# leggedrobotics/wild_visual_navigation

Hardware: AMD Instinct MI355X
Metric: frames/sec (448x448 DINO-ViT-S/8 + seg + MLP train-step) (higher is better)
Workload: dtype fp16 + e5m2-MX-correction linears (a w = a_h w_h + 2^-12 (a_h8 w_l8 + a_l8 w_h8); ~16 significand bits per product) + f16 attention products (two-plane q in the first six blocks), fp32 accumulate / residual (<= 1e-3 parity mode)

## Files before the change

### include/wvn_hip.h

```cpp
#ifndef WVN_HIP_H
#define WVN_HIP_H
#include <stddef.h>
#ifdef __cplusplus
extern "C" {
#endif

#define WVN_MAX_DEPTH 32
#define WVN_PREC_F32 0
#define WVN_PREC_BF16 1
#define WVN_PREC_X3 2
#define WVN_PREC_FP8 3
#define WVN_PREC_F16 4

#define WVN_PREC_MIX 5

int wvn_version(void);

#define WVN_VIT_MLP_FUSED 1
#define WVN_VIT_QKV_FUSED 2
#define WVN_VIT_FUSE_ANY_SIZE 4
#define WVN_VIT_NO_PROJ_IN_MLP 8
#define WVN_VIT_NO_LN_HANDOVER 16
#define WVN_VIT_NO_A384_X3 32
#define WVN_VIT_X3_NO_A384 64
// ... 251 lines not shown
int wvn_pixel_mlp_pack(const wvn_mlp_desc* d, const float* params, void* packed, void* stream);
int wvn_pixel_mlp_infer(const wvn_mlp_desc* d, const void* packed, void* zx, int ldzx, int batch, int grid, int out_h,
                        int out_w, float mean, float std, float std_factor, const float* conf_state, float* trav,
                        float* conf, float* loss_reco, void* stream);

size_t wvn_pixel_mlp_exact_pack_bytes(const wvn_mlp_desc* d);
size_t wvn_pixel_mlp_exact_workspace_bytes(const wvn_mlp_desc* d, int batch, int grid);
int wvn_pixel_mlp_exact_pack(const wvn_mlp_desc* d, const float* params, void* packed, void* stream);
int wvn_pixel_mlp_infer_exact(const wvn_mlp_desc* d, const float* params, const void* packed, const float* tokens,
                              int ld_tokens, int batch, int grid, int out_h, int out_w, float mean, float std,
                              float std_factor, const float* conf_state, float* trav, float* conf, float* loss_reco,
                              void* workspace, size_t workspace_bytes, void* stream);

size_t wvn_segment_predict_workspace_bytes(const wvn_mlp_desc* d, int B, int S);
int wvn_segment_predict(const wvn_mlp_desc* d, const float* params, const float* feat, int ld_row, long long ld_frame,
                        int B, int S, const void* seg, int seg_bytes, int H, int W, float mean, float std, float std_factor,
                        const float* conf_state, float* trav, float* conf, float* loss_reco, void* workspace,
                        size_t workspace_bytes, void* stream);

size_t wvn_wire_bytes(int H, int W, int S, int D);
int wvn_wire_pack(const void* seg, int seg_is_i64, const float* feat, int ldf, void* out, int H, int W, int S, int D, void* stream);
int wvn_wire_unpack(const void* in, long long* seg_i64, int* seg_i32, float* feat, int H, int W, int S, int D, void* stream);

int wvn_debug_gemm_bf16_timed(const void* A, int lda, const void* W, int ldw, const float* bias, void* C, int ldc, int M,
                              int N, int K, int epi, long long* dbg, void* stream);
int wvn_debug_gemm_a384_x3(const void* A, const void* A_lo, int lda, const void* W, const void* W_lo, const float* bias, void* C,
                           void* C_lo, int ldc, int M, int N, int epi, long long* dbg, void* stream);
int wvn_debug_gemm_n384_x3(const void* A, const void* A_lo, int lda, const void* W, const void* W_lo, const float* bias, const float* ls,
                           float* C, int ldc, int M, int K, long long* dbg, void* stream);
int wvn_debug_mlp_x3_frag(const void* xn, const void* xn_lo, const void* W1, const void* W1_lo, const float* b1, void* hid, void* hid_lo,
                          const void* W2p, const float* b2, float* x, int M, int F, long long* dbg1, long long* dbg2, void* stream);
int wvn_debug_gemm_n384_mx(const void* A_h, const void* A_l8, const void* A_h8, const void* Wp, const float* bias, const float* ls, float* C,
                           int ldc, int M, int K, long long* dbg, void* stream);
int wvn_debug_mlp_mx(const float* x, int ldx, const float* ln_stats, const float* ln_g, const float* ln_b, const void* W1p, const float* b1,
                     void* hid_h, void* hid_l8, void* hid_h8, const void* W2p, const float* b2, float* xout, int M, int F, long long* dbg1,
                     long long* dbg2, void* stream);
int wvn_debug_qkv_mx(const float* x, int ldx, const float* ln_stats, const float* ln_g, const float* ln_b, const void* Wp, const float* bias, void* q,
                     void* q_lo, void* k, void* vt, int heads, int npad, int ntok_s, float q_scale, int M, long long* dbg, void* stream);
int wvn_debug_f16_saturate(const float* in, void* out_f16, int n, void* stream);
int wvn_debug_attention_timing(long long* dbg);
int wvn_debug_attention_variant(int variant);
int wvn_debug_attention_planes(const void* q, const void* q_lo, const void* k, const void* vt, void* out, void* out_lo, int B, int heads,
                               int ntok, int ntok_s, int npad, int out_frag, int qsplit_form, void* stream);
int wvn_debug_n384_pair(int on);
int wvn_debug_kmeans_assign_form(int form);
int wvn_debug_kmeans_linear_rows(int rows);

int wvn_debug_kmeans_screen_stats(unsigned long long* out, int reset);
int wvn_debug_qkv_fused_timing(long long* dbg);
int wvn_debug_mlp_fused_timing(long long* dbg);
int wvn_debug_gemm_n384(const void* A, int lda, const void* W, int ldw, const float* bias, float* C, int ldc, int M, int K,
                        void* stream);


size_t wvn_dense_crf_workspace_bytes(int B, int H, int W, int K);
int wvn_dense_crf(const float* logits1, int K1, long long s1b, long long s1c, long long s1p, const float* logits2, int K2, long long s2b,
                  long long s2c, long long s2p, const unsigned char* image, int B, int H, int W, int iterations, float pos_w, float pos_xy_std,
                  float bi_w, float bi_xy_std, float bi_rgb_std, int* labels, int* nseg_last, float* probs, float* debug, void* workspace,
                  size_t workspace_bytes, void* stream);
int wvn_crf_image(const void* frame, int frame_u8, int B, int src_h, int src_w, const int* rows, const int* cols, int out_h, int out_w,
                  unsigned char* out, void* stream);

size_t wvn_dense_crf_permutohedral_workspace_bytes(int B, int H, int W, int K);
int wvn_dense_crf_permutohedral(const float* logits1, int K1, long long s1b, long long s1c, long long s1p, const float* logits2, int K2,
                                long long s2b, long long s2c, long long s2p, const unsigned char* image, int B, int H, int W, int iterations,
                                float pos_w, float pos_xy_std, float bi_w, float bi_xy_std, float bi_rgb_std, int* labels, int* nseg_last,
// ... 12 lines not shown
```

### wild_visual_navigation_amd/_lib.py

```python
import ctypes as C
import os
import threading

import torch

_HERE = os.path.dirname(os.path.abspath(__file__))
LIB_PATH = os.environ.get("WVN_LIB_PATH") or os.path.join(_HERE, "lib", "libwvn_hip.so")
if os.environ.get("WVN_LIB_PATH"):
    import sys as _sys

    print(f"[wild_visual_navigation_amd] WVN_LIB_PATH is set: loading {LIB_PATH} instead of the in-tree build", file=_sys.stderr)

WVN_MAX_DEPTH = 32
PREC_F32, PREC_BF16, PREC_X3, PREC_FP8, PREC_F16, PREC_MIX = 0, 1, 2, 3, 4, 5
VIT_MLP_FUSED = 1
VIT_QKV_FUSED = 2
VIT_FUSE_ANY_SIZE = 4
VIT_NO_PROJ_IN_MLP = 8
VIT_NO_LN_HANDOVER = 16
VIT_NO_A384_X3 = 32
VIT_NO_MX = 1024


def vit_qsplit_blocks(n: int) -> int:
# ... 33 lines not shown
        ("mlp_dim", C.c_int), ("precision", C.c_int), ("flags", C.c_int),
        ("patch_w", C.c_void_p), ("patch_b", C.c_void_p), ("cls_pos", C.c_void_p), ("pos", C.c_void_p),
        ("norm_g", C.c_void_p), ("norm_b", C.c_void_p),
        ("layers", VitLayer * WVN_MAX_DEPTH),
    ]


class MlpDesc(C.Structure):
    _fields_ = [("D", C.c_int), ("H1", C.c_int), ("H2", C.c_int), ("reserved", C.c_int)]


_lib = None
_lock = threading.Lock()

_i, _f, _p, _ll, _sz = C.c_int, C.c_float, C.c_void_p, C.c_longlong, C.c_size_t
_SIGNATURES = {
    "wvn_version": ([], _i),
    "wvn_vit_workspace_bytes": ([_p, _i], _sz),
    "wvn_vit_forward": ([_p, _p, _i, _p, _p, _i, _p, _sz, _p], _i),
    "wvn_vit_forward_u8": ([_p, _p, _i, _p, _p, _i, _p, _sz, _p], _i),
    "wvn_vit_forward_frames": ([_p, _p, _i, _i, _i, _p, _p, _i, _p, _p, _i, _p, _sz, _p], _i),
    "wvn_vit_forward_frames_pair": ([_p, _p, _i, _i, _i, _p, _p, _p, _i, _p, _p, _i, _p, _sz, _p], _i),
    "wvn_resize_nearest_crop": ([_p, _p, _ll, _i, _i, _p, _p, _i, _i, _i, _p], _i),
    "wvn_prof_enable": ([_i], _i),
    "wvn_prof_collect": ([_p, _p], _i),
    "wvn_gemm_bf16": ([_p, _i, _p, _i, _p, _p, _i, _i, _i, _i, _i, _p], _i),
    "wvn_debug_attention_variant": ([_i], _i),
    "wvn_debug_attention_planes": ([_p, _p, _p, _p, _p, _p, _i, _i, _i, _i, _i, _i, _i, _p], _i),
    "wvn_debug_kmeans_assign_form": ([_i], _i),
    "wvn_debug_kmeans_screen_stats": ([_p, _i], _i),
    "wvn_debug_mlp_x3_frag": ([_p, _p, _p, _p, _p, _p, _p, _p, _p, _p, _i, _i, _p, _p, _p], _i),
    "wvn_debug_gemm_n384_x3": ([_p, _p, _i, _p, _p, _p, _p, _p, _i, _i, _i, _p, _p], _i),
    "wvn_debug_gemm_n384_mx": ([_p, _p, _p, _p, _p, _p, _p, _i, _i, _i, _p, _p], _i),
    "wvn_debug_mlp_mx": ([_p, _i, _p, _p, _p, _p, _p, _p, _p, _p, _p, _p, _p, _i, _i, _p, _p, _p], _i),
    "wvn_debug_qkv_mx": ([_p, _i, _p, _p, _p, _p, _p, _p, _p, _p, _p, _i, _i, _i, _f, _i, _p, _p], _i),
    "wvn_debug_gemm_a384_x3": ([_p, _p, _i, _p, _p, _p, _p, _p, _i, _i, _i, _i, _p, _p], _i),
    "wvn_stream_create_cu_mask": ([_p, _p, _i], _i),
    "wvn_stream_destroy": ([_p], _i),
    "wvn_debug_qkv_fused_timing": ([_p], _i),
    "wvn_debug_mlp_fused_timing": ([_p], _i),
    "wvn_qkv_fused": ([_p, _i, _p, _p, _f, _p, _p, _p, _p, _p, _i, _i, _i, _f, _i, _p], _i),
    "wvn_proj_mlp_fused": ([_p, _i, _p, _p, _p, _p, _p, _f, _p, _p, _p, _p, _p, _p, _i, _i, _i, _p], _i),
    "wvn_mlp_fused": ([_p, _i, _p, _p, _f, _p, _p, _p, _p, _p, _p, _i, _i, _i, _p], _i),
    "wvn_gemm_f16": ([_p, _i, _p, _i, _p, _p, _i, _i, _i, _i, _i, _p], _i),
    "wvn_qkv_fused_f16": ([_p, _i, _p, _p, _f, _p, _p, _p, _p, _p, _i, _i, _i, _f, _i, _p], _i),
    "wvn_proj_mlp_resident": ([_p, _i, _p, _p, _p, _p, _f, _p, _p, _p, _p, _p, _i, _i, _i, _p, _p, _f, _p, _p], _i),
    "wvn_proj_mlp_resident_f16": ([_p, _i, _p, _p, _p, _p, _f, _p, _p, _p, _p, _p, _i, _i, _i, _p, _p, _f, _p, _p], _i),
    "wvn_qkv_prenorm": ([_p, _p, _p, _p, _p, _p, _i, _i, _i, _f, _i, _p], _i),
    "wvn_qkv_prenorm_f16": ([_p, _p, _p, _p, _p, _p, _i, _i, _i, _f, _i, _p], _i),
    "wvn_proj_mlp_fused_f16": ([_p, _i, _p, _p, _p, _p, _p, _f, _p, _p, _p, _p, _p, _p, _i, _i, _i, _p], _i),
    "wvn_mlp_fused_f16": ([_p, _i, _p, _p, _f, _p, _p, _p, _p, _p, _p, _i, _i, _i, _p], _i),
    "wvn_attention_f16": ([_p, _p, _p, _p, _i, _i, _i, _i, _f, _p], _i),
    "wvn_gemm_x3": ([_p, _p, _i, _p, _p, _i, _p, _p, _p, _i, _i, _i, _i, _i, _p], _i),
    "wvn_quantize_rows_fp8": ([_p, _i, _i, _p, _i, _p, _i, _i, _p], _i),
    "wvn_layernorm_fp8": ([_p, _p, _p, _p, _i, _p, _i, _i, _f, _p], _i),
    "wvn_gemm_fp8": ([_p, _i, _p, _i, _p, _p, _p, _p, _i, _i, _i, _i, _i, _p], _i),
    "wvn_gemm_a768_fp8": ([_p, _i, _p, _p, _p, _p, _p, _p, _i, _i, _i, _i, _p, _p, _p, _i, _i, _i, _f, _p], _i),
    "wvn_gemm_fp8_mx": ([_p, _i, _p, _p, _i, _p, _p, _p, _p, _i, _i, _i, _i, _i, _p], _i),
    "wvn_split_planes": ([_p, _i, _p, _p, _i, _i, _i, _p], _i),
    "wvn_attention_x3": ([_p, _p, _p, _p, _p, _p, _p, _p, _i, _i, _i, _i, _f, _p], _i),
    "wvn_gemm_f32": ([_p, _i, _i, _p, _i, _i, _p, _p, _i, _i, _i, _i, _i, _p, _i, _p], _i),
    "wvn_layernorm": ([_p, _p, _p, _p, _i, _i, _i, _f, _p], _i),
    "wvn_attention_bf16": ([_p, _p, _p, _p, _i, _i, _i, _i, _f, _p], _i),
    "wvn_attention_f32": ([_p, _p, _p, _p, _i, _i, _i, _i, _f, _p], _i),
    "wvn_patchify": ([_p, _p, _i, _i, _i, _i, _p], _i),
    "wvn_patchify_u8": ([_p, _p, _i, _i, _i, _p], _i),
# ... 109 lines not shown
```

### wild_visual_navigation_amd/csrc/api.hip

```cpp
#include <math.h>
#include <string.h>

#include "../../include/wvn_hip.h"

#include "common.h"
#include "wvn_internal.h"

#define RET_IF(x)            \
  do {                       \
    int rc__ = (x);          \
    if (rc__ != WVN_OK) return rc__; \
  } while (0)

extern "C" {

int wvn_version(void) { return 100; }

size_t wvn_vit_workspace_bytes(const wvn_vit_model* m, int batch) {
  if (!m || batch <= 0) return 0;
  return wvn_vit_workspace_bytes_impl(m, batch);
}

int wvn_vit_forward(const wvn_vit_model* m, const float* img, int batch, float* tokens_f32, void* tokens_lowp,
                    int ld_lowp, void* workspace, size_t workspace_bytes, void* stream) {
// ... 175 lines not shown
int wvn_debug_qkv_fused_timing(long long* dbg) { g_qkv_fused_dbg = dbg; return WVN_OK; }
int wvn_stream_create_cu_mask(void** stream, const unsigned int* mask, int words) {
  if (!stream || !mask || words <= 0) return WVN_ERR_ARG;
  hipStream_t st = nullptr;
  const hipError_t e = hipExtStreamCreateWithCUMask(&st, (uint32_t)words, mask);
  if (e != hipSuccess) return (int)e;
  *stream = (void*)st;
  return WVN_OK;
}
int wvn_stream_destroy(void* stream) {
  if (!stream) return WVN_ERR_ARG;
  const hipError_t e = hipStreamDestroy((hipStream_t)stream);
  return e == hipSuccess ? WVN_OK : (int)e;
}

int wvn_debug_gemm_a384_x3(const void* A, const void* A_lo, int lda, const void* W, const void* W_lo, const float* bias, void* C,
                           void* C_lo, int ldc, int M, int N, int epi, long long* dbg, void* stream) {
  if (epi != EPI_GELU_BF16 && epi != EPI_RESID_F32) return WVN_ERR_ARG;
  return wvn_gemm_a384_x3_launch(wvn_desc_a384(A, A_lo, lda, W, W_lo, bias, C, C_lo, ldc, M, N, dbg), epi, (hipStream_t)stream);
}
int wvn_debug_gemm_n384_x3(const void* A, const void* A_lo, int lda, const void* W, const void* W_lo, const float* bias, const float* ls,
                           float* C, int ldc, int M, int K, long long* dbg, void* stream) {
  return wvn_gemm_n384_x3_launch(wvn_desc_n384(A, A_lo, lda, W, W_lo, bias, ls, C, ldc, M, K, nullptr, dbg), EPI_RESID_F32, (hipStream_t)stream);
}
int wvn_debug_mlp_x3_frag(const void* xn, const void* xn_lo, const void* W1, const void* W1_lo, const float* b1, void* hid, void* hid_lo,
                          const void* W2p, const float* b2, float* x, int M, int F, long long* dbg1, long long* dbg2, void* stream) {
  RET_IF(wvn_gemm_a384_x3_launch(wvn_desc_a384(xn, xn_lo, 384, W1, W1_lo, b1, hid, hid_lo, F, M, F, dbg1), EPI_GELU_FRAG, (hipStream_t)stream));
  return wvn_gemm_n384_x3_frag_launch(wvn_desc_n384(hid, hid_lo, F, W2p, nullptr, b2, nullptr, x, 384, M, F, nullptr, dbg2), EPI_RESID_F32, (hipStream_t)stream);
}
int wvn_debug_gemm_n384_mx(const void* A_h, const void* A_l8, const void* A_h8, const void* Wp, const float* bias, const float* ls, float* C,
                           int ldc, int M, int K, long long* dbg, void* stream) {
  return wvn_gemm_n384_mx_launch(wvn_desc_n384(A_h, A_l8, K, Wp, nullptr, bias, ls, C, ldc, M, K, nullptr, dbg, A_h8), EPI_RESID_F32, (hipStream_t)stream);
}
int wvn_debug_mlp_mx(const float* x, int ldx, const float* ln_stats, const float* ln_g, const float* ln_b, const void* W1p, const float* b1,
                     void* hid_h, void* hid_l8, void* hid_h8, const void* W2p, const float* b2, float* xout, int M, int F, long long* dbg1,
                     long long* dbg2, void* stream) {
  GemmBf16Params p1 = wvn_desc_a384(nullptr, nullptr, 0, W1p, nullptr, b1, hid_h, hid_l8, F, M, F, dbg1, hid_h8);
  wvn_desc_ln_on_load(p1, x, ldx, ln_stats, ln_g, ln_b);
  RET_IF(wvn_gemm_a384_mx_launch(p1, EPI_GELU_FRAG, (hipStream_t)stream));
  if (!W2p) return WVN_OK;
  return wvn_gemm_n384_mx_launch(wvn_desc_n384(hid_h, hid_l8, F, W2p, nullptr, b2, nullptr, xout, 384, M, F, nullptr, dbg2, hid_h8), EPI_RESID_F32, (hipStream_t)stream);
}
int wvn_debug_qkv_mx(const float* x, int ldx, const float* ln_stats, const float* ln_g, const float* ln_b, const void* Wp, const float* bias, void* q,
                     void* q_lo, void* k, void* vt, int heads, int npad, int ntok_s, float q_scale, int M, long long* dbg, void* stream) {
  GemmBf16Params p = wvn_desc_a384(nullptr, nullptr, 0, Wp, nullptr, bias, nullptr, nullptr, 0, M, 3 * heads * 64, dbg);
  wvn_desc_ln_on_load(p, x, ldx, ln_stats, ln_g, ln_b);
  wvn_desc_qkv_epilogue(p, q, k, vt, heads, npad, 0, ntok_s, q_scale, 1, q_lo);
  return wvn_gemm_a384_mx_launch(p, EPI_QKV, (hipStream_t)stream);
}
int wvn_debug_n384_pair(int on) {
  if (on >= 32) { wvn_gemm_a384_mx_set_form(on - 32); return WVN_OK; }
  wvn_gemm_n384_x3_set_pair(on);
  return WVN_OK;
}
int wvn_debug_kmeans_screen_stats(unsigned long long* out, int reset) { return out ? wvn_kmeans_pixels_screen_stats(out, reset) : WVN_ERR_ARG; }
int wvn_debug_kmeans_assign_form(int form) { wvn_kmeans_pixels_set_assign_form(form); return WVN_OK; }
int wvn_debug_attention_variant(int v) { wvn_attention_bf16_set_variant(v); wvn_attention_bf16_set_variant_f16(v); return WVN_OK; }
int wvn_debug_attention_planes(const void* q, const void* q_lo, const void* k, const void* vt, void* out, void* out_lo, int B, int heads, int ntok,
                               int ntok_s, int npad, int out_frag, int qsplit_form, void* stream) {
  if (!q || !k || !vt || !out || B < 1 || heads < 1 || ntok < 1 || ntok_s < ntok || ntok_s > npad) return WVN_ERR_ARG;
  if (qsplit_form < 0 || qsplit_form > 2 || (qsplit_form == 0) != (q_lo == nullptr)) return WVN_ERR_ARG;
  if (out_frag < 0 || out_frag > 2 || (out_frag != 0 && (!out_lo || heads != 6))) return WVN_ERR_ARG;
  return wvn_attention_bf16_launch_f16((const bf16_t*)q, (const bf16_t*)k, (const bf16_t*)vt, (bf16_t*)out, B, heads, ntok, ntok_s, npad, 0.f,
                                       (hipStream_t)stream, (bf16_t*)out_lo, (const bf16_t*)q_lo, out_frag, qsplit_form);
}

int wvn_debug_gemm_bf16_timed(const void* A, int lda, const void* W, int ldw, const float* bias, void* C, int ldc, int M,
                              int N, int K, int epi, long long* dbg, void* stream) {
  if (epi < 0 || epi > EPI_ACCUM_F32 || !C) return WVN_ERR_ARG;
  GemmBf16Params p{};
  p.A = (const bf16_t*)A; p.lda = lda; p.W = (const bf16_t*)W; p.ldw = ldw; p.bias = bias; p.C = C; p.ldc = ldc;
  p.M = M; p.N = N; p.K = K; p.dbg = dbg;
  return wvn_gemm_bf16_launch(p, epi, (hipStream_t)stream);
}

int wvn_debug_gemm_n384(const void* A, int lda, const void* W, int ldw, const float* bias, float* C, int ldc, int M, int K,
                        void* stream) {
  GemmBf16Params p{};
  p.A = (const bf16_t*)A; p.lda = lda; p.W = (const bf16_t*)W; p.ldw = ldw; p.bias = bias; p.C = C; p.ldc = ldc;
  p.M = M; p.N = 384; p.K = K;
  return wvn_gemm_n384_launch(p, EPI_RESID_F32, (hipStream_t)stream, nullptr, 1);
}

// ... 421 lines not shown
```

### wild_visual_navigation_amd/csrc/gemm_n384_x3.hip

```cpp
#include <type_traits>

#include "common.h"
#include "wvn_internal.h"

namespace {

constexpr int NN = 384;
constexpr int NTILE = NN / 32;
constexpr int BKS = 16;
constexpr int BM = 128;
constexpr int NS = 4;
constexpr int W_PLANE = NN * BKS * 2;
constexpr int A_PLANE = BM * BKS * 2;
constexpr int A_OFF = 2 * W_PLANE;
constexpr int STAGE_BYTES = 2 * W_PLANE + 2 * A_PLANE;
constexpr int RING_BYTES = NS * STAGE_BYTES;
constexpr int STG_PITCH = 132;
constexpr int STG_BYTES = 32 * STG_PITCH * 4;
constexpr int BIAS_OFF = RING_BYTES;
constexpr int LS_OFF = BIAS_OFF + NN * 4;
constexpr int LDS_BYTES = LS_OFF + NN * 4;
constexpr int WP = 6, AP = 2;

struct N384X3Params {
// ... 529 lines not shown
            __builtin_amdgcn_sched_group_barrier(0x008, 1, 0);
            __builtin_amdgcn_sched_group_barrier(0x100, 1, 0);
            __builtin_amdgcn_sched_group_barrier(0x010, 1, 0);
            __builtin_amdgcn_sched_group_barrier(0x002, 2, 0);
          }
          __builtin_amdgcn_sched_barrier(0);
        }
        if (i + PD < nk) load_a(i + PD, jj);
        __builtin_amdgcn_sched_barrier(0);
        if constexpr (TIMING) { t_wait += c1 - c0; t_steps += (long long)__builtin_amdgcn_s_memtime() - c1; }
      }
    }
    long long e0 = 0;
    if constexpr (TIMING) e0 = (long long)__builtin_amdgcn_s_memtime();
    asm volatile("s_waitcnt vmcnt(0)" ::: "memory");
    n384_pair_epilogue(acc, smem, wave, lane, rg, ch, m0w, rs_c, p.ldc, bias_l, ls_l, p.stats, p.eps, p.M);
    if constexpr (TIMING) t_epi += (long long)__builtin_amdgcn_s_memtime() - e0;
  }
  if constexpr (TIMING) {
    if (lane == 0 && p.dbg && ch == 0) {
      long long* d = p.dbg + ((size_t)blockIdx.x * 4 + rg) * 4;
      d[0] = t_wait; d[1] = t_steps; d[2] = t_epi; d[3] = (long long)__builtin_amdgcn_s_memtime() - t_start;
    }
  }
}

typedef __attribute__((ext_vector_type(8))) int i32x8_t;
typedef __attribute__((ext_vector_type(8))) _Float16 f16x8_t;
constexpr int MXD = 2;
constexpr int MX_SC_ONE = 0x7f7f7f7f, MX_SC_RES = 0x73737373;

struct N384MXExtra { unsigned a_l8_off; };

template <bool TIMING, int VAR = 0>
__global__ __launch_bounds__(512, 1) void gemm_n384_mx_pair_kernel(N384X3Params p, N384MXExtra ex) {
  wvn_fp16_saturate();
  extern __shared__ __attribute__((aligned(16))) unsigned char smem[];
  const int tid = threadIdx.x, lane = tid & 63;
  const int wave = __builtin_amdgcn_readfirstlane(tid >> 6);
  const int rg = wave & 3, ch = wave >> 2;
  const int l31 = lane & 31, hi = lane >> 5;
  const int nk = p.K / BKS;
  const int nmac = p.K / 64;
  const float* bias_l = (const float*)(smem + PBIAS_OFF);
  const float* ls_l = (const float*)(smem + PLS_OFF);
  for (int i = tid; i < NN; i += 512) {
    ((float*)(smem + PBIAS_OFF))[i] = p.bias ? p.bias[i] : 0.f;
    ((float*)(smem + PLS_OFF))[i] = p.ls ? p.ls[i] : 1.f;
  }
  const __amdgpu_buffer_rsrc_t rs_w = __builtin_amdgcn_make_buffer_rsrc((void*)p.W, 0, (unsigned)((size_t)4 * NN * p.K), 0x00020000);
  const size_t mpad = (size_t)(p.M + 31) / 32 * 32;
  const __amdgpu_buffer_rsrc_t rs_a = __builtin_amdgcn_make_buffer_rsrc((void*)p.A, 0, (unsigned)(ex.a_l8_off + mpad * p.K), 0x00020000);
  const __amdgpu_buffer_rsrc_t rs_c = __builtin_amdgcn_make_buffer_rsrc((void*)p.C, 0, (unsigned)((size_t)p.M * p.ldc * 4), 0x00020000);
  const unsigned wv0 = (unsigned)(wave * PFW * 1024 + lane * 16);
  const unsigned rdw = l31 * 32 + ((hi ^ ((l31 >> 3) & 1)) << 4) + ch * 6 * 1024;

  long long t_wait = 0, t_steps = 0, t_epi = 0;
  const long long t_start = TIMING ? (long long)__builtin_amdgcn_s_memtime() : 0;
  const int nrb = (p.M + BM - 1) / BM;
  for (int rb = blockIdx.x; rb < nrb; rb += gridDim.x) {
    const int m0w = rb * BM + rg * 32;
    const unsigned a_base = __builtin_amdgcn_readfirstlane((unsigned)((size_t)(m0w >> 5) * p.K * 64));
    const unsigned a8_base = __builtin_amdgcn_readfirstlane((unsigned)((size_t)(m0w >> 5) * p.K * 32));
    auto piece_w = [&](int i, int u) {
      unsigned char* st = smem + (i % PNS) * FSTAGE;
      __builtin_amdgcn_raw_ptr_buffer_load_lds(rs_w, (__attribute__((address_space(3))) void*)(st + (wave * PFW + u) * 1024), 16, wv0 + u * 1024,
                                               __builtin_amdgcn_readfirstlane((unsigned)i * FSTAGE), 0, 0);
    };
    u32x4_t ah[MXD][4], a8[MXD][2][2];
    auto load_ah = [&](int c, int slot) {
#pragma unroll
      for (int s = 0; s < 4; ++s)
        ah[slot][s] = __builtin_amdgcn_raw_buffer_load_b128(rs_a, lane * 16, __builtin_amdgcn_readfirstlane(a_base + (unsigned)(c * 4 + s) * 1024), 0);
    };
    auto load_a8 = [&](int c, int slot) {
#pragma unroll
      for (int x = 0; x < 2; ++x)
        a8[slot][1][x] = __builtin_amdgcn_raw_buffer_load_b128(rs_a, lane * 16, __builtin_amdgcn_readfirstlane(a8_base + ex.a_l8_off + (unsigned)(c * 2 + x) * 1024), 0);
    };
    auto derive_h8 = [&](int slot) {
      typedef __attribute__((ext_vector_type(2))) short s16x2_t;
      typedef __attribute__((ext_vector_type(2))) _Float16 h2_t;
#pragma unroll
      for (int sfr = 0; sfr < 4; ++sfr) {
        uint32_t d[2] = {0, 0};
#pragma unroll
        for (int e = 0; e < 4; ++e) {
          const uint32_t pr = ah[slot][sfr][e];
          const s16x2_t o = __builtin_bit_cast(s16x2_t, d[e >> 1]);
          d[e >> 1] = __builtin_bit_cast(uint32_t, (e & 1) ? __builtin_amdgcn_cvt_scalef32_pk_bf8_f16(o, __builtin_bit_cast(h2_t, pr), 1.0f, true)
                                                           : __builtin_amdgcn_cvt_scalef32_pk_bf8_f16(o, __builtin_bit_cast(h2_t, pr), 1.0f, false));
        }
        a8[slot][0][sfr >> 1][2 * (sfr & 1)] = d[0];
        a8[slot][0][sfr >> 1][2 * (sfr & 1) + 1] = d[1];
      }
    };
    __syncthreads();
#pragma unroll
    for (int c = 0; c < MXD; ++c) {
      load_ah(c, c);
      __builtin_amdgcn_sched_barrier(0);
      load_a8(c, c);
      __builtin_amdgcn_sched_barrier(0);
    }
#pragma unroll
    for (int i0 = 0; i0 < PNS - 1; ++i0)
      if (i0 < nk) {
#pragma unroll
        for (int u = 0; u < PFW; ++u) piece_w(i0, u);
      }

    f32x16_t acc[NTILE / 2];
#pragma unroll
    for (int t = 0; t < NTILE / 2; ++t)
#pragma unroll
      for (int r = 0; r < 16; ++r) acc[t][r] = 0.f;

    u32x4_t wq[2][2][2];
    asm volatile("s_waitcnt vmcnt(%0)" ::"n"((PNS - 2) * PFW) : "memory");
    __builtin_amdgcn_s_barrier();
#pragma unroll
    for (int x = 0; x < 2; ++x)
#pragma unroll
      for (int t = 0; t < 2; ++t) wq[0][x][t] = *(const u32x4_t*)(smem + rdw + x * W_PLANE + t * 1024);
    for (int ib = 0; ib < nk; ib += 4 * MXD) {
#pragma unroll
      for (int jj = 0; jj < 4 * MXD; ++jj) {
        const int i = ib + jj;
        const int kind = jj & 3, slot = jj >> 2;
        long long c0 = 0, c1 = 0;
        if constexpr (TIMING) c0 = (long long)__builtin_amdgcn_s_memtime();
        if constexpr (VAR != 4) {
          constexpr int W3 = (PNS - 3) * PFW;
          if (jj == 0) { if (i == 0) asm volatile("s_waitcnt vmcnt(%0)" ::"n"(W3) : "memory"); else asm volatile("s_waitcnt vmcnt(%0)" ::"n"(W3 + 6) : "memory"); }
          else if (jj == 1) { if (i == 1) asm volatile("s_waitcnt vmcnt(%0)" ::"n"(W3) : "memory"); else asm volatile("s_waitcnt vmcnt(%0)" ::"n"(W3 + 2) : "memory"); }
          else if (jj == 2) { if (i == 2) asm volatile("s_waitcnt vmcnt(%0)" ::"n"(W3 + 4) : "memory"); else asm volatile("s_waitcnt vmcnt(%0)" ::"n"(W3 + 6) : "memory"); }
          else if ((jj & 3) == 0) asm volatile("s_waitcnt vmcnt(%0)" ::"n"(W3 + 6) : "memory");
          else if ((jj & 3) == 1) asm volatile("s_waitcnt vmcnt(%0)" ::"n"(W3 + 2) : "memory");
          else if ((jj & 3) == 2) asm volatile("s_waitcnt vmcnt(%0)" ::"n"(W3 + 6) : "memory");
          else asm volatile("s_waitcnt vmcnt(%0)" ::"n"(W3 + 4) : "memory");
          __builtin_amdgcn_s_barrier();
        }
        if constexpr (TIMING) c1 = (long long)__builtin_amdgcn_s_memtime();
        __builtin_amdgcn_sched_barrier(0);
        const unsigned char* st = smem + (i % PNS) * FSTAGE;
        const unsigned char* st1 = smem + ((i + 1) % PNS) * FSTAGE;
        const int s0 = jj & 1;
#pragma unroll
        for (int pr = 0; pr < NTILE / 4; ++pr) {
          const int cur = (s0 + pr) & 1, nx = cur ^ 1;
          if constexpr (!(VAR & 1) || VAR == 4) piece_w(i + PNS - 1, pr);
          const unsigned char* src = pr + 1 < NTILE / 4 ? st + (2 * pr + 2) * 1024 : st1;
#pragma unroll
          for (int x = 0; x < 2; ++x)
#pragma unroll
            for (int t = 0; t < 2; ++t) wq[nx][x][t] = *(const u32x4_t*)(src + rdw + x * W_PLANE + t * 1024);
          if (kind == 1 && pr == 0) derive_h8(slot);
          if (kind < 2) {
#pragma unroll
            for (int x = 0; x < 2; ++x)
#pragma unroll
              for (int t = 0; t < 2; ++t)
                acc[2 * pr + t] = __builtin_amdgcn_mfma_f32_32x32x16_f16(__builtin_bit_cast(f16x8_t, wq[cur][x][t]), __builtin_bit_cast(f16x8_t, ah[slot][2 * kind + x]),
                                                                         acc[2 * pr + t], 0, 0, 0);
#pragma unroll
            for (int n = 0; n < 4; ++n) {
              __builtin_amdgcn_sched_group_barrier(0x008, 1, 0);
              __builtin_amdgcn_sched_group_barrier(0x100, 1, 0);
              __builtin_amdgcn_sched_group_barrier(0x010, 1, 0);
              __builtin_amdgcn_sched_group_barrier(0x002, 2, 0);
            }
          } else {
            const u32x4_t a0 = a8[slot][kind - 2][0], a1 = a8[slot][kind - 2][1];
            const i32x8_t av = {(int)a0[0], (int)a0[1], (int)a0[2], (int)a0[3], (int)a1[0], (int)a1[1], (int)a1[2], (int)a1[3]};
#pragma unroll
            for (int t = 0; t < 2; ++t) {
              const u32x4_t w0 = wq[cur][0][t], w1 = wq[cur][1][t];
              const i32x8_t wv = {(int)w0[0], (int)w0[1], (int)w0[2], (int)w0[3], (int)w1[0], (int)w1[1], (int)w1[2], (int)w1[3]};
              acc[2 * pr + t] = __builtin_amdgcn_mfma_scale_f32_32x32x64_f8f6f4(wv, av, acc[2 * pr + t], 1, 1, 0, kind == 2 ? MX_SC_RES : MX_SC_ONE, 0,
                                                                                kind == 2 ? MX_SC_ONE : MX_SC_RES);
            }
#pragma unroll
            for (int n = 0; n < 2; ++n) {
              __builtin_amdgcn_sched_group_barrier(0x008, 1, 0);
              __builtin_amdgcn_sched_group_barrier(0x100, 2, 0);
              __builtin_amdgcn_sched_group_barrier(0x010, 1, 0);
              __builtin_amdgcn_sched_group_barrier(0x002, 4, 0);
            }
          }
          __builtin_amdgcn_sched_barrier(0);
        }
        const int c2 = (i >> 2) + MXD;
        if constexpr (!(VAR & 2) || VAR == 4) {
          if (kind == 1) load_ah(c2, slot);
          if (kind == 3) load_a8(c2, slot);
        }
        __builtin_amdgcn_sched_barrier(0);
        if constexpr (TIMING) { t_wait += c1 - c0; t_steps += (long long)__builtin_amdgcn_s_memtime() - c1; }
      }
    }
    long long e0 = 0;
    if constexpr (TIMING) e0 = (long long)__builtin_amdgcn_s_memtime();
    asm volatile("s_waitcnt vmcnt(0)" ::: "memory");
    n384_pair_epilogue(acc, smem, wave, lane, rg, ch, m0w, rs_c, p.ldc, bias_l, ls_l, p.stats, p.eps, p.M);
    if constexpr (TIMING) t_epi += (long long)__builtin_amdgcn_s_memtime() - e0;
  }
  if constexpr (TIMING) {
    if (lane == 0 && p.dbg && ch == 0) {
      long long* d = p.dbg + ((size_t)blockIdx.x * 4 + rg) * 4;
      d[0] = t_wait; d[1] = t_steps; d[2] = t_epi; d[3] = (long long)__builtin_amdgcn_s_memtime() - t_start;
    }
  }
}

int g_n384_mx_var = 0;
int g_n384_pair = 1;

int n384x3_num_cus() {
  static int n = 0;
  if (n == 0) {
    int dev = 0;
    hipDeviceProp_t prop;
    if (hipGetDevice(&dev) == hipSuccess && hipGetDeviceProperties(&prop, dev) == hipSuccess) n = prop.multiProcessorCount;
    if (n <= 0) n = 256;
  }
  return n;
}

}

int wvn_gemm_n384_x3_launch(const GemmBf16Params& g, int epi, hipStream_t st) {
  const bool patch = epi == EPI_PATCH;
  if (epi != EPI_RESID_F32 && epi != EPI_ACCUM_F32 && !patch) return WVN_ERR_ARG;
  if (patch && (!g.pos || g.npatch <= 0 || (g.npatch & 1) || g.ntok_s < g.npatch + 1 || g.ldc != NN || g.ls || (g.M % g.npatch) != 0)) return WVN_ERR_ARG;
  if (g.N != NN || g.K <= 0 || (g.K % BKS) != 0 || g.M <= 0 || !g.A || !g.A_lo || !g.W || !g.W_lo || !g.C) return WVN_ERR_ARG;
  if ((g.lda % 8) || (g.ldw % 8) || (g.ldc % 4) || g.ldw != g.K) return WVN_ERR_ARG;
  if (((uintptr_t)g.A | (uintptr_t)g.A_lo | (uintptr_t)g.W | (uintptr_t)g.W_lo | (uintptr_t)g.C) & 15) return WVN_ERR_ARG;
  if (g.A_lo <= g.A || g.W_lo <= g.W) return WVN_ERR_ARG;
  const size_t a_plane = (size_t)(g.A_lo - g.A), w_plane = (size_t)(g.W_lo - g.W);
  const size_t c_rows = patch ? (size_t)(g.M / g.npatch) * g.ntok_s : (size_t)g.M;
  if ((a_plane + (size_t)g.M * g.lda) * 2 >= (1ull << 32) || c_rows * g.ldc * 4 >= (1ull << 32) || (w_plane + (size_t)NN * g.ldw) * 2 >= (1ull << 32))
    return WVN_ERR_ARG;
  N384X3Params p{};
  p.A = g.A; p.a_plane = a_plane; p.lda = g.lda; p.W = g.W; p.w_plane = w_plane; p.ldw = g.ldw; p.bias = g.bias; p.ls = g.ls;
  p.C = (float*)g.C; p.ldc = g.ldc; p.M = g.M; p.K = g.K; p.dbg = g.dbg; p.stats = g.ln_stats_out; p.eps = g.ln_eps;
  if (patch) { p.pos = g.pos; p.npatch = g.npatch; p.ntok_s = g.ntok_s; p.c_rows = (int)c_rows; p.stats = nullptr; }
  static LdsOptIn lds_opt_in;
  if (const int rc = lds_opt_in(LDS_BYTES, (const void*)gemm_n384_x3_kernel<false>, (const void*)gemm_n384_x3_kernel<true>)) return rc;
// ... 14 lines not shown
  if ((a_plane + mpad * g.K) * 2 >= (1ull << 32) || (size_t)g.M * g.ldc * 4 >= (1ull << 32) || (size_t)2 * NN * g.K * 2 >= (1ull << 31)) return WVN_ERR_ARG;
  N384X3Params p{};
  p.A = g.A; p.a_plane = a_plane; p.lda = g.K; p.W = g.W; p.w_plane = 0; p.ldw = g.K; p.bias = g.bias; p.ls = g.ls;
  p.C = (float*)g.C; p.ldc = g.ldc; p.M = g.M; p.K = g.K; p.dbg = g.dbg; p.stats = g.ln_stats_out; p.eps = g.ln_eps;
  static LdsOptIn lds_opt_in;
  if (const int rc = lds_opt_in(PAIR_LDS_BYTES, (const void*)gemm_n384_x3_frag_kernel<false>, (const void*)gemm_n384_x3_frag_kernel<true>,
                                (const void*)gemm_n384_x3_frag_pair_kernel<false>, (const void*)gemm_n384_x3_frag_pair_kernel<true>)) return rc;
  const int ncu = n384x3_num_cus(), nrb = ceil_div(g.M, BM);
  const int grid = nrb < ncu ? nrb : ncu;
  if (g_n384_pair) {
    if (p.dbg) hipLaunchKernelGGL(gemm_n384_x3_frag_pair_kernel<true>, dim3(grid), dim3(512), PAIR_LDS_BYTES, st, p);
    else hipLaunchKernelGGL(gemm_n384_x3_frag_pair_kernel<false>, dim3(grid), dim3(512), PAIR_LDS_BYTES, st, p);
  } else if (p.dbg) hipLaunchKernelGGL(gemm_n384_x3_frag_kernel<true>, dim3(grid), dim3(256), LDS_BYTES, st, p);
  else hipLaunchKernelGGL(gemm_n384_x3_frag_kernel<false>, dim3(grid), dim3(256), LDS_BYTES, st, p);
  WVN_LAUNCH_CHECK();
  return WVN_OK;
}
int wvn_gemm_n384_mx_launch(const GemmBf16Params& g, int epi, hipStream_t st) {
  if (epi != EPI_RESID_F32 && epi != EPI_ACCUM_F32) return WVN_ERR_ARG;
  if (g.N != NN || g.K <= 0 || (g.K % 128) != 0 || g.M <= 0 || !g.A || !g.A_lo || !g.W || !g.C || (g.ldc % 4)) return WVN_ERR_ARG;
  if (((uintptr_t)g.A | (uintptr_t)g.A_lo | (uintptr_t)g.W | (uintptr_t)g.C) & 15) return WVN_ERR_ARG;
  const size_t mpad = (size_t)(g.M + 31) / 32 * 32;
  const uintptr_t a0 = (uintptr_t)g.A, al = (uintptr_t)g.A_lo;
  if (al < a0 + mpad * g.K * 2) return WVN_ERR_ARG;
  const uintptr_t top = al + mpad * g.K;
  if (top - a0 >= (1ull << 32) || (size_t)g.M * g.ldc * 4 >= (1ull << 32) || (size_t)4 * NN * g.K >= (1ull << 31)) return WVN_ERR_ARG;
  N384X3Params p{};
  p.A = g.A; p.a_plane = 0; p.lda = g.K; p.W = g.W; p.w_plane = 0; p.ldw = g.K; p.bias = g.bias; p.ls = g.ls;
  p.C = (float*)g.C; p.ldc = g.ldc; p.M = g.M; p.K = g.K; p.dbg = g.dbg; p.stats = g.ln_stats_out; p.eps = g.ln_eps;
  N384MXExtra ex{(unsigned)(al - a0)};
  static LdsOptIn lds_opt_in;
  if (const int rc = lds_opt_in(PAIR_LDS_BYTES, (const void*)gemm_n384_mx_pair_kernel<false>, (const void*)gemm_n384_mx_pair_kernel<true>,
                                (const void*)gemm_n384_mx_pair_kernel<true, 1>, (const void*)gemm_n384_mx_pair_kernel<true, 2>,
                                (const void*)gemm_n384_mx_pair_kernel<true, 3>, (const void*)gemm_n384_mx_pair_kernel<true, 4>)) return rc;
  const int ncu = n384x3_num_cus(), nrb = ceil_div(g.M, BM);
  const int grid = nrb < ncu ? nrb : ncu;
  if (p.dbg && g_n384_mx_var == 1) hipLaunchKernelGGL((gemm_n384_mx_pair_kernel<true, 1>), dim3(grid), dim3(512), PAIR_LDS_BYTES, st, p, ex);
  else if (p.dbg && g_n384_mx_var == 2) hipLaunchKernelGGL((gemm_n384_mx_pair_kernel<true, 2>), dim3(grid), dim3(512), PAIR_LDS_BYTES, st, p, ex);
  else if (p.dbg && g_n384_mx_var == 3) hipLaunchKernelGGL((gemm_n384_mx_pair_kernel<true, 3>), dim3(grid), dim3(512), PAIR_LDS_BYTES, st, p, ex);
  else if (p.dbg && g_n384_mx_var == 4) hipLaunchKernelGGL((gemm_n384_mx_pair_kernel<true, 4>), dim3(grid), dim3(512), PAIR_LDS_BYTES, st, p, ex);
  else if (p.dbg) hipLaunchKernelGGL(gemm_n384_mx_pair_kernel<true>, dim3(grid), dim3(512), PAIR_LDS_BYTES, st, p, ex);
  else hipLaunchKernelGGL(gemm_n384_mx_pair_kernel<false>, dim3(grid), dim3(512), PAIR_LDS_BYTES, st, p, ex);
  WVN_LAUNCH_CHECK();
  return WVN_OK;
}
void wvn_gemm_n384_x3_set_pair(int on) {
  if (on >= 16) { g_n384_mx_var = on - 16; return; }
  g_n384_pair = on ? 1 : 0;
}
```

### wild_visual_navigation_amd/csrc/wvn_internal.h

```cpp
#pragma once
#include "common.h"

enum GemmEpilogue {
  EPI_BF16 = 0,
  EPI_GELU_BF16 = 1,
  EPI_RELU_BF16 = 2,
  EPI_F32 = 3,
  EPI_RESID_F32 = 4,
  EPI_ACCUM_F32 = 5,
  EPI_PATCH = 6,
  EPI_QKV = 7,
  EPI_GELU_MX8 = 9,
  EPI_GELU_FRAG = 8,
};

struct GemmBf16Params {
  const bf16_t* A; int lda;
  const bf16_t* W; int ldw;
  const float* bias;
  void* C; int ldc;
  int M, N, K;
  const float* pos; int npatch; int ntok;
  int ntok_s;
  bf16_t* q; bf16_t* k; bf16_t* vt; int heads; int npad;
// ... 126 lines not shown
int wvn_attention_x3_launch(const bf16_t* q_hi, const bf16_t* q_lo, const bf16_t* k_hi, const bf16_t* k_lo, const bf16_t* vt_hi,
                            const bf16_t* vt_lo, bf16_t* out_hi, bf16_t* out_lo, int B, int heads, int ntok, int ntok_s,
                            int npad, float scale, hipStream_t st);

int wvn_splitk_reduce_launch(const float* part, int splitk, size_t n, const float* bias, int ncols, float* out,
                             hipStream_t st);
int wvn_upsample_bilinear_launch(const float* tok, float* out, int B, int G, int D, int H, hipStream_t st);
int wvn_upsample_nearest_i32_launch(const int* lab, int* out, int B, int G, int H, hipStream_t st);
int wvn_segpool_launch(const int* seg, const float* tok, int ldf, float* feat, void* W, int* cnt, int B, int H,
                       int Wd, int G, int S, int D, hipStream_t st);
int wvn_label_pool_batched_launch(const void* nodes, int n, int C, int H, int Wd, int Smax, long long* sum, int* cnt,
                                  hipStream_t st);
int wvn_label_pool_launch(const float* mask, int C, const int* seg, float* signal, unsigned char* valid, void* sum,
                          int* cnt, int H, int Wd, int S, hipStream_t st);
int wvn_centers_launch(const int* seg, float* centers, unsigned long long* scratch, int H, int Wd, int S,
                       hipStream_t st);
int wvn_adjacency_launch(const int* seg, long long* edges, int* count, unsigned char* bitmap, int H, int Wd, int S,
                         int max_edges, hipStream_t st);
int wvn_normalize_rows_launch(const float* code, int ldc, float* xn, int rows, int C, hipStream_t st);
int wvn_argmax_rows_launch(const float* x, int ld, int rows, int cols, int* out, hipStream_t st);
size_t wvn_kmeans_scratch_floats(int B, int P, int C, int K);
size_t wvn_kmeans_pixels_scratch_floats(int B, int G, int H, int C, int K);
int wvn_kmeans_pixels_launch(const float* code, int* labels, int* nseg, float* scratch, int B, int G, int H, int C, int K, int iters,
                             int relabel, hipStream_t st);
int wvn_km_pix_prepare_launch(const float* code, float* rinv, float* cent, int B, int G, int H, int C, int K, hipStream_t st, int align_corners = 1);
int wvn_km_relabel_launch(int* labels, int* nseg, int B, long long P, int K, int relabel, hipStream_t st);
int wvn_kmeans_pixels_linear_supported(int G, int H, int C, int K);
size_t wvn_kmeans_pixels_linear_scratch_floats(int B, int G, int H, int C, int K);
void wvn_kmeans_pixels_linear_set_rows(int rc);
int wvn_kmeans_pixels_linear_launch(const float* code, int* labels, int* nseg, float* scratch, int B, int G, int H, int C, int K,
                                    int iters, int relabel, hipStream_t st, int align_corners = 1);
int wvn_f16_saturate_probe_launch(const float* in, uint16_t* out, int n, hipStream_t st);
void wvn_gemm_n384_x3_set_pair(int on);
void wvn_gemm_a384_mx_set_form(int form);
int wvn_table_slots(int K);
int wvn_table_bilerp_argmax_launch(const float* table, int* labels, int B, int G, int H, int K, hipStream_t st, int align_corners = 1);
void wvn_kmeans_pixels_set_assign_form(int form);
int wvn_kmeans_pixels_screen_stats(unsigned long long* out, int reset);
int wvn_flip_average_launch(const float* a, const float* mirrored, float* out, int B, int G, int C, hipStream_t st);
int wvn_kmeans_launch(const float* xn, int* labels, int* nseg, float* scratch, int B, int P, int C, int K, int iters,
                      int relabel, hipStream_t st);
struct ConfArgs {
  int method = 0;
  int balanced = 1;
  double* state = nullptr;
  float* minmax = nullptr;
};
int wvn_mlp_rowloss_stats_launch(const float* out, int ldo, const float* x, int ldx, const unsigned char* valid,
                                 float* lr, double* stats, int R, int D, hipStream_t st, const int* rows_dev = nullptr,
                                 const ConfArgs& conf = ConfArgs());
int wvn_compact_segment_rows_launch(const float* feat, int D, const float* side, int Ds, const int* nseg, int B, int S, float* x,
                                    float* side_out, int* count, hipStream_t st);
bool wvn_mlp_train_fused_ok(int D, int H1, int H2, int R);
size_t wvn_mlp_train_fused_scratch_bytes(int R);
int wvn_mlp_train_fwd_launch(const float* P, const size_t* off, size_t ntotal, const float* x, int ldx, const unsigned char* valid, int R,
                             int D, const int* rows_dev, float* h1, float* h2, float* out, float* lr, double* stats, void* scratch,
                             unsigned* sync_word, hipStream_t st, const ConfArgs& conf = ConfArgs());
int wvn_mlp_train_bwd_launch(const float* P, const size_t* off, size_t ntotal, const float* x, int ldx, const float* y,
                             const unsigned char* valid, int R, int D, const int* rows_dev, float* h1, float* h2, float* out, float* lr,
                             float* g_out, float* g_h2, float* g_h1, const double* stats, float std_factor, float w_trav, float w_reco,
                             float* conf_out, float* grads, void* scratch, hipStream_t st, const ConfArgs& conf = ConfArgs());
int wvn_mlp_gradout_launch(const float* out, int ldo, const float* x, int ldx, const float* y,
                           const unsigned char* valid, const float* lr, const double* stats, float std_factor,
                           float w_trav, float w_reco, float* g, int ldg, float* trav_w, float* trav_raw,
                           float* conf_out, float* extra, int R, int D, hipStream_t st, const int* rows_dev = nullptr,
                           const ConfArgs& conf = ConfArgs());
// ... 48 lines not shown
```

Before: 883.8.

## Stage n384 MX GEMM A operand through LDS window once per block

Adds an AONCE variant of the n384 MX pair GEMM kernel that loads the A operand (high and low-fp8 planes) with asynchronous buffer-to-LDS loads into a window carved out of the shared ring. The W ring depth drops from PNS to ANS stages to make room. A fragments are then read from LDS instead of loaded straight into registers, and the waitcnt/barrier schedule is rewritten to match. AONCE is enabled by default, and debug entry points expose the last kernel form and a stats path. The aim is to cut A-operand global-load latency and register pressure in the main loop. The cost is a shallower W prefetch ring and extra LDS reads and barriers.

```diff
diff --git a/include/wvn_hip.h b/include/wvn_hip.h
--- a/include/wvn_hip.h
+++ b/include/wvn_hip.h
@@ -307,6 +307,9 @@
                           const void* W2p, const float* b2, float* x, int M, int F, long long* dbg1, long long* dbg2, void* stream);
 int wvn_debug_gemm_n384_mx(const void* A_h, const void* A_l8, const void* A_h8, const void* Wp, const float* bias, const float* ls, float* C,
                            int ldc, int M, int K, long long* dbg, void* stream);
+int wvn_debug_gemm_n384_mx_stats(const void* A_h, const void* A_l8, const void* Wp, const float* bias, const float* ls, float* C, int ldc, int M, int K,
+                                 float* ln_stats_out, void* stream);
+int wvn_debug_n384_mx_last_form(void);
 int wvn_debug_mlp_mx(const float* x, int ldx, const float* ln_stats, const float* ln_g, const float* ln_b, const void* W1p, const float* b1,
                      void* hid_h, void* hid_l8, void* hid_h8, const void* W2p, const float* b2, float* xout, int M, int F, long long* dbg1,
                      long long* dbg2, void* stream);
diff --git a/wild_visual_navigation_amd/_lib.py b/wild_visual_navigation_amd/_lib.py
--- a/wild_visual_navigation_amd/_lib.py
+++ b/wild_visual_navigation_amd/_lib.py
@@ -89,6 +89,8 @@
     "wvn_debug_mlp_x3_frag": ([_p, _p, _p, _p, _p, _p, _p, _p, _p, _p, _i, _i, _p, _p, _p], _i),
     "wvn_debug_gemm_n384_x3": ([_p, _p, _i, _p, _p, _p, _p, _p, _i, _i, _i, _p, _p], _i),
     "wvn_debug_gemm_n384_mx": ([_p, _p, _p, _p, _p, _p, _p, _i, _i, _i, _p, _p], _i),
+    "wvn_debug_n384_mx_last_form": ([], _i),
+    "wvn_debug_gemm_n384_mx_stats": ([_p, _p, _p, _p, _p, _p, _i, _i, _i, _p, _p], _i),
     "wvn_debug_mlp_mx": ([_p, _i, _p, _p, _p, _p, _p, _p, _p, _p, _p, _p, _p, _i, _i, _p, _p, _p], _i),
     "wvn_debug_qkv_mx": ([_p, _i, _p, _p, _p, _p, _p, _p, _p, _p, _p, _i, _i, _i, _f, _i, _p, _p], _i),
     "wvn_debug_gemm_a384_x3": ([_p, _p, _i, _p, _p, _p, _p, _p, _i, _i, _i, _i, _p, _p], _i),
diff --git a/wild_visual_navigation_amd/csrc/api.hip b/wild_visual_navigation_amd/csrc/api.hip
--- a/wild_visual_navigation_amd/csrc/api.hip
+++ b/wild_visual_navigation_amd/csrc/api.hip
@@ -231,6 +231,11 @@
                            int ldc, int M, int K, long long* dbg, void* stream) {
   return wvn_gemm_n384_mx_launch(wvn_desc_n384(A_h, A_l8, K, Wp, nullptr, bias, ls, C, ldc, M, K, nullptr, dbg, A_h8), EPI_RESID_F32, (hipStream_t)stream);
 }
+int wvn_debug_gemm_n384_mx_stats(const void* A_h, const void* A_l8, const void* Wp, const float* bias, const float* ls, float* C, int ldc, int M, int K,
+                                 float* ln_stats_out, void* stream) {
+  return wvn_gemm_n384_mx_launch(wvn_desc_n384(A_h, A_l8, K, Wp, nullptr, bias, ls, C, ldc, M, K, ln_stats_out), EPI_RESID_F32, (hipStream_t)stream);
+}
+int wvn_debug_n384_mx_last_form(void) { return wvn_gemm_n384_mx_last_form(); }
 int wvn_debug_mlp_mx(const float* x, int ldx, const float* ln_stats, const float* ln_g, const float* ln_b, const void* W1p, const float* b1,
                      void* hid_h, void* hid_l8, void* hid_h8, const void* W2p, const float* b2, float* xout, int M, int F, long long* dbg1,
                      long long* dbg2, void* stream) {
@@ -248,6 +253,7 @@
   return wvn_gemm_a384_mx_launch(p, EPI_QKV, (hipStream_t)stream);
 }
 int wvn_debug_n384_pair(int on) {
+  if (on >= 64) { wvn_gemm_n384_x3_set_pair(on); return WVN_OK; }
   if (on >= 32) { wvn_gemm_a384_mx_set_form(on - 32); return WVN_OK; }
   wvn_gemm_n384_x3_set_pair(on);
   return WVN_OK;
diff --git a/wild_visual_navigation_amd/csrc/gemm_n384_x3.hip b/wild_visual_navigation_amd/csrc/gemm_n384_x3.hip
--- a/wild_visual_navigation_amd/csrc/gemm_n384_x3.hip
+++ b/wild_visual_navigation_amd/csrc/gemm_n384_x3.hip
@@ -585,8 +585,14 @@
 
 struct N384MXExtra { unsigned a_l8_off; };
 
-template <bool TIMING, int VAR = 0>
+constexpr int ANS = 5;
+constexpr int AWIN_OFF = ANS * FSTAGE;
+constexpr int AWIN_RG = 6 * 1024;
+static_assert(AWIN_OFF + 4 * AWIN_RG <= PRING_BYTES && 8 * PSTG_BYTES <= AWIN_OFF, "A window inside the shipped ring, behind the staging images");
+
+template <bool TIMING, int VAR = 0, bool AONCE = false>
 __global__ __launch_bounds__(512, 1) void gemm_n384_mx_pair_kernel(N384X3Params p, N384MXExtra ex) {
+  constexpr int RNS = AONCE ? ANS : PNS;
   wvn_fp16_saturate();
   extern __shared__ __attribute__((aligned(16))) unsigned char smem[];
   const int tid = threadIdx.x, lane = tid & 63;
@@ -616,11 +622,21 @@
     const unsigned a_base = __builtin_amdgcn_readfirstlane((unsigned)((size_t)(m0w >> 5) * p.K * 64));
     const unsigned a8_base = __builtin_amdgcn_readfirstlane((unsigned)((size_t)(m0w >> 5) * p.K * 32));
     auto piece_w = [&](int i, int u) {
-      unsigned char* st = smem + (i % PNS) * FSTAGE;
+      unsigned char* st = smem + (i % RNS) * FSTAGE;
       __builtin_amdgcn_raw_ptr_buffer_load_lds(rs_w, (__attribute__((address_space(3))) void*)(st + (wave * PFW + u) * 1024), 16, wv0 + u * 1024,
                                                __builtin_amdgcn_readfirstlane((unsigned)i * FSTAGE), 0, 0);
     };
     u32x4_t ah[MXD][4], a8[MXD][2][2];
+    auto piece_a = [&](unsigned so, int q, int base) {
+      __builtin_amdgcn_raw_ptr_buffer_load_lds(rs_a, (__attribute__((address_space(3))) void*)(smem + base + rg * AWIN_RG + q * 1024), 16, lane * 16,
+                                               __builtin_amdgcn_readfirstlane(so), 0, 0);
+    };
+    auto piece_ah = [&](int c, int base) {
+      piece_a(a_base + (unsigned)(c * 4 + 2 * ch) * 1024, 2 * ch, base);
+      piece_a(a_base + (unsigned)(c * 4 + 2 * ch + 1) * 1024, 2 * ch + 1, base);
+    };
+    auto piece_al = [&](int c, int base) { piece_a(a8_base + ex.a_l8_off + (unsigned)(c * 2 + ch) * 1024, 4 + ch, base); };
+    auto read_a = [&](int q, int base) { return *(const u32x4_t*)(smem + base + rg * AWIN_RG + q * 1024 + lane * 16); };
     auto load_ah = [&](int c, int slot) {
 #pragma unroll
       for (int s = 0; s < 4; ++s)
@@ -649,19 +665,39 @@
       }
     };
     __syncthreads();
-#pragma unroll
-    for (int c = 0; c < MXD; ++c) {
-      load_ah(c, c);
+    if constexpr (!AONCE) {
+#pragma unroll
+      for (int c = 0; c < MXD; ++c) {
+        load_ah(c, c);
+        __builtin_amdgcn_sched_barrier(0);
+        load_a8(c, c);
+        __builtin_amdgcn_sched_barrier(0);
+      }
+    } else {
+      constexpr int S4 = (ANS - 1) * FSTAGE;
+      piece_ah(0, AWIN_OFF); piece_al(1, AWIN_OFF);
+      piece_ah(1, S4); piece_al(0, S4);
       __builtin_amdgcn_sched_barrier(0);
-      load_a8(c, c);
+    }
+#pragma unroll
+    for (int i0 = 0; i0 < RNS - 1; ++i0)
+      if (i0 < nk) {
+#pragma unroll
+        for (int u = 0; u < PFW; ++u) piece_w(i0, u);
+      }
+    if constexpr (AONCE) {
       __builtin_amdgcn_sched_barrier(0);
-    }
-#pragma unroll
-    for (int i0 = 0; i0 < PNS - 1; ++i0)
-      if (i0 < nk) {
-#pragma unroll
-        for (int u = 0; u < PFW; ++u) piece_w(i0, u);
-      }
+      asm volatile("s_waitcnt vmcnt(%0)" ::"n"((ANS - 1) * PFW) : "memory");
+      __builtin_amdgcn_s_barrier();
+      __builtin_amdgcn_sched_barrier(0);
+      constexpr int S4 = (ANS - 1) * FSTAGE;
+#pragma unroll
+      for (int s = 0; s < 4; ++s) { ah[0][s] = read_a(s, AWIN_OFF); ah[1][s] = read_a(s, S4); }
+#pragma unroll
+      for (int x = 0; x < 2; ++x) { a8[0][1][x] = read_a(4 + x, S4); a8[1][1][x] = read_a(4 + x, AWIN_OFF); }
+      __builtin_amdgcn_sched_barrier(0);
+      asm volatile("s_waitcnt lgkmcnt(0)" ::: "memory");
+    }
 
     f32x16_t acc[NTILE / 2];
 #pragma unroll
@@ -670,8 +706,13 @@
       for (int r = 0; r < 16; ++r) acc[t][r] = 0.f;
 
     u32x4_t wq[2][2][2];
-    asm volatile("s_waitcnt vmcnt(%0)" ::"n"((PNS - 2) * PFW) : "memory");
+    asm volatile("s_waitcnt vmcnt(%0)" ::"n"((RNS - 2) * PFW) : "memory");
     __builtin_amdgcn_s_barrier();
+    if constexpr (AONCE) {
+      __builtin_amdgcn_sched_barrier(0);
+      piece_ah(2, AWIN_OFF);
+      __builtin_amdgcn_sched_barrier(0);
+    }
 #pragma unroll
     for (int x = 0; x < 2; ++x)
 #pragma unroll
@@ -683,7 +724,12 @@
         const int kind = jj & 3, slot = jj >> 2;
         long long c0 = 0, c1 = 0;
         if constexpr (TIMING) c0 = (long long)__builtin_amdgcn_s_memtime();
-        if constexpr (VAR != 4) {
+        if constexpr (VAR != 4 && AONCE) {
+          constexpr int W2 = (ANS - 3) * PFW;
+          if (kind < 2) asm volatile("s_waitcnt vmcnt(%0)" ::"n"(W2 + 2) : "memory");
+          else asm volatile("s_waitcnt vmcnt(%0)" ::"n"(W2 + 1) : "memory");
+          __builtin_amdgcn_s_barrier();
+        } else if constexpr (VAR != 4) {
           constexpr int W3 = (PNS - 3) * PFW;
           if (jj == 0) { if (i == 0) asm volatile("s_waitcnt vmcnt(%0)" ::"n"(W3) : "memory"); else asm volatile("s_waitcnt vmcnt(%0)" ::"n"(W3 + 6) : "memory"); }
           else if (jj == 1) { if (i == 1) asm volatile("s_waitcnt vmcnt(%0)" ::"n"(W3) : "memory"); else asm volatile("s_waitcnt vmcnt(%0)" ::"n"(W3 + 2) : "memory"); }
@@ -696,13 +742,23 @@
         }
         if constexpr (TIMING) c1 = (long long)__builtin_amdgcn_s_memtime();
         __builtin_amdgcn_sched_barrier(0);
-        const unsigned char* st = smem + (i % PNS) * FSTAGE;
-        const unsigned char* st1 = smem + ((i + 1) % PNS) * FSTAGE;
+        const unsigned char* st = smem + (i % RNS) * FSTAGE;
+        const unsigned char* st1 = smem + ((i + 1) % RNS) * FSTAGE;
         const int s0 = jj & 1;
 #pragma unroll
         for (int pr = 0; pr < NTILE / 4; ++pr) {
           const int cur = (s0 + pr) & 1, nx = cur ^ 1;
-          if constexpr (!(VAR & 1) || VAR == 4) piece_w(i + PNS - 1, pr);
+          if constexpr (!(VAR & 1) || VAR == 4) piece_w(i + RNS - 1, pr);
+          if constexpr (AONCE && (!(VAR & 2) || VAR == 4)) {
+            if (pr == 0 && kind == 2) {
+#pragma unroll
+              for (int s = 0; s < 4; ++s) ah[slot][s] = read_a(s, AWIN_OFF);
+            }
+            if (pr == 0 && kind == 0) {
+#pragma unroll
+              for (int x = 0; x < 2; ++x) a8[slot ^ 1][1][x] = read_a(4 + x, AWIN_OFF);
+            }
+          }
           const unsigned char* src = pr + 1 < NTILE / 4 ? st + (2 * pr + 2) * 1024 : st1;
 #pragma unroll
           for (int x = 0; x < 2; ++x)
@@ -744,7 +800,12 @@
           __builtin_amdgcn_sched_barrier(0);
         }
         const int c2 = (i >> 2) + MXD;
-        if constexpr (!(VAR & 2) || VAR == 4) {
+        if constexpr (AONCE) {
+          if constexpr (!(VAR & 2) || VAR == 4) {
+            if (kind == 1) piece_al(c2, AWIN_OFF);
+            if (kind == 3) piece_ah(c2 + 1, AWIN_OFF);
+          }
+        } else if constexpr (!(VAR & 2) || VAR == 4) {
           if (kind == 1) load_ah(c2, slot);
           if (kind == 3) load_a8(c2, slot);
         }
@@ -767,6 +828,8 @@
 }
 
 int g_n384_mx_var = 0;
+int g_n384_mx_last = -1;
+int g_n384_mx_aonce = 1;
 int g_n384_pair = 1;
 
 int n384x3_num_cus() {
@@ -847,10 +910,21 @@
   static LdsOptIn lds_opt_in;
   if (const int rc = lds_opt_in(PAIR_LDS_BYTES, (const void*)gemm_n384_mx_pair_kernel<false>, (const void*)gemm_n384_mx_pair_kernel<true>,
                                 (const void*)gemm_n384_mx_pair_kernel<true, 1>, (const void*)gemm_n384_mx_pair_kernel<true, 2>,
-                                (const void*)gemm_n384_mx_pair_kernel<true, 3>, (const void*)gemm_n384_mx_pair_kernel<true, 4>)) return rc;
+                                (const void*)gemm_n384_mx_pair_kernel<true, 3>, (const void*)gemm_n384_mx_pair_kernel<true, 4>,
+                                (const void*)gemm_n384_mx_pair_kernel<false, 0, true>, (const void*)gemm_n384_mx_pair_kernel<true, 0, true>,
+                                (const void*)gemm_n384_mx_pair_kernel<true, 1, true>, (const void*)gemm_n384_mx_pair_kernel<true, 2, true>,
+                                (const void*)gemm_n384_mx_pair_kernel<true, 3, true>, (const void*)gemm_n384_mx_pair_kernel<true, 4, true>)) return rc;
   const int ncu = n384x3_num_cus(), nrb = ceil_div(g.M, BM);
   const int grid = nrb < ncu ? nrb : ncu;
-  if (p.dbg && g_n384_mx_var == 1) hipLaunchKernelGGL((gemm_n384_mx_pair_kernel<true, 1>), dim3(grid), dim3(512), PAIR_LDS_BYTES, st, p, ex);
+  g_n384_mx_last = g_n384_mx_aonce;
+  if (g_n384_mx_aonce) {
+    if (p.dbg && g_n384_mx_var == 1) hipLaunchKernelGGL((gemm_n384_mx_pair_kernel<true, 1, true>), dim3(grid), dim3(512), PAIR_LDS_BYTES, st, p, ex);
+    else if (p.dbg && g_n384_mx_var == 2) hipLaunchKernelGGL((gemm_n384_mx_pair_kernel<true, 2, true>), dim3(grid), dim3(512), PAIR_LDS_BYTES, st, p, ex);
+    else if (p.dbg && g_n384_mx_var == 3) hipLaunchKernelGGL((gemm_n384_mx_pair_kernel<true, 3, true>), dim3(grid), dim3(512), PAIR_LDS_BYTES, st, p, ex);
+    else if (p.dbg && g_n384_mx_var == 4) hipLaunchKernelGGL((gemm_n384_mx_pair_kernel<true, 4, true>), dim3(grid), dim3(512), PAIR_LDS_BYTES, st, p, ex);
+    else if (p.dbg) hipLaunchKernelGGL((gemm_n384_mx_pair_kernel<true, 0, true>), dim3(grid), dim3(512), PAIR_LDS_BYTES, st, p, ex);
+    else hipLaunchKernelGGL((gemm_n384_mx_pair_kernel<false, 0, true>), dim3(grid), dim3(512), PAIR_LDS_BYTES, st, p, ex);
+  } else if (p.dbg && g_n384_mx_var == 1) hipLaunchKernelGGL((gemm_n384_mx_pair_kernel<true, 1>), dim3(grid), dim3(512), PAIR_LDS_BYTES, st, p, ex);
   else if (p.dbg && g_n384_mx_var == 2) hipLaunchKernelGGL((gemm_n384_mx_pair_kernel<true, 2>), dim3(grid), dim3(512), PAIR_LDS_BYTES, st, p, ex);
   else if (p.dbg && g_n384_mx_var == 3) hipLaunchKernelGGL((gemm_n384_mx_pair_kernel<true, 3>), dim3(grid), dim3(512), PAIR_LDS_BYTES, st, p, ex);
   else if (p.dbg && g_n384_mx_var == 4) hipLaunchKernelGGL((gemm_n384_mx_pair_kernel<true, 4>), dim3(grid), dim3(512), PAIR_LDS_BYTES, st, p, ex);
@@ -859,7 +933,9 @@
   WVN_LAUNCH_CHECK();
   return WVN_OK;
 }
+int wvn_gemm_n384_mx_last_form() { return g_n384_mx_last; }
 void wvn_gemm_n384_x3_set_pair(int on) {
+  if (on >= 64) { g_n384_mx_aonce = on > 64 ? 1 : 0; return; }
   if (on >= 16) { g_n384_mx_var = on - 16; return; }
   g_n384_pair = on ? 1 : 0;
 }
diff --git a/wild_visual_navigation_amd/csrc/wvn_internal.h b/wild_visual_navigation_amd/csrc/wvn_internal.h
--- a/wild_visual_navigation_amd/csrc/wvn_internal.h
+++ b/wild_visual_navigation_amd/csrc/wvn_internal.h
@@ -182,6 +182,7 @@
                                     int iters, int relabel, hipStream_t st, int align_corners = 1);
 int wvn_f16_saturate_probe_launch(const float* in, uint16_t* out, int n, hipStream_t st);
 void wvn_gemm_n384_x3_set_pair(int on);
+int wvn_gemm_n384_mx_last_form();
 void wvn_gemm_a384_mx_set_form(int form);
 int wvn_table_slots(int K);
 int wvn_table_bilerp_argmax_launch(const float* table, int* labels, int B, int G, int H, int K, hipStream_t st, int align_corners = 1);
```

Result: no change. 892.2, median of 6 (+1.0%).
